# LoveDaisy/ice_halo_sim

Hardware: AMD Instinct MI355X
Metric: rays/sec (whole node) at 9 wavelengths, single-scatter hex column (higher is better)
Workload: dtype f32

## Files before the change

### ice_halo_sim_amd/csrc/halo_backend.cpp

```cpp
#include <cstdlib>
#include <dlfcn.h>
#include <hip/hip_runtime.h>

#include <algorithm>
#include <cmath>
#include <cstdio>
#include <cstring>
#include <map>
#include <memory>
#include <mutex>
#include <string>
#include <vector>

#include "halo_device.h"
#include "halo_host.hpp"
#include "halo_launch.h"

#ifndef HALO_XYZ_LOG_MIN_PIX
#define HALO_XYZ_LOG_MIN_PIX (1u << 19)
#endif

using namespace halo;

namespace {
// ... 47 lines not shown
  int mono_enabled = 1;
  int bin = -1;
  DevBuf<HitRec> bin_list_s[2], bin_list2_s[2];
  DevBuf<uint32_t> bin_cnt_s[2], bin_cnt2_s[2];
  int log_set = 0;
  Marker set_free[2];
  hipStream_t aux = nullptr;
  hipEvent_t ev_fork = nullptr, ev_join = nullptr;
  bool aux_pending = false;
  hipStream_t cs[2] = {nullptr, nullptr};
  hipEvent_t ev_cs[2] = {nullptr, nullptr}, ev_main = nullptr, ev_aux = nullptr;
  bool cs_pending[2] = {false, false};
  int cs_next = 0;
  uint64_t aux_seq = 0, cs_seen_aux[2] = {0, 0};
  int overlap = 1;
  int defer_fold = 0;
  int twin_set = 0;
  int lambda_planes = -1;
  int mono_copies = 8;
  uint32_t mono_s_log2 = 0;
  int blocks_per_cu = 24;
  int host_shapes = 0;
  int gen_serial = 0;
  int small_blocks_per_cu = 0;
  int blocks_cap = 0;
  int lazy_fold = 1;
  int hit_log = -1;
  uint32_t hit_log_cap = 0;
  int hex_fast = 1;
  int entry_fast = 1;
// ... 100 lines not shown
  uint64_t cont_in_n = 0;
  int cont_shuffle = 1;
  int cont_order = 0;
  DevBuf<uint32_t> cont_mask;
  DevBuf<uint32_t> cont_err;
  DevBuf<uint32_t> cont_base;
  DevBuf<uint32_t> cont_tiles;
  uint32_t cont_fill_max = 0;
  uint64_t cont_roots = 0;
  DevBuf<HaloExitRecord> exits;
  uint64_t exits_pending = 0;
  DevBuf<float> host_f;
  DevBuf<uint32_t> host_u;
  uint64_t sess_crystal_samples = 0, sess_orient_samples = 0;
  std::vector<hipEvent_t*> untimed_events() {
    return {&ev_cs[0], &ev_cs[1], &ev_main, &ev_aux, &ev_fork, &ev_join, &ev_gen, &ev_gate, &set_free[0].ev, &set_free[1].ev, &shapes_free[0].ev,
            &shapes_free[1].ev, &rmw[0].ev, &rmw[1].ev, &set_folded[0].ev, &set_folded[1].ev};
  }
};

namespace {

int fail(HaloBackend* b, int code, const std::string& msg) {
  if (b) b->error = msg;
  return code;
}
int hip_fail(HaloBackend* b, hipError_t e, const char* what) {
  return fail(b, (e == hipErrorNoDevice || e == hipErrorInvalidDevice || e == hipErrorOutOfMemory) ? HALO_UNAVAILABLE : HALO_FATAL,
              std::string(what) + ": " + hipGetErrorString(e));
}
#define HIPCHK(b, call)                                   \
// ... 17 lines not shown
  b->aux_seq++;
  return HALO_OK;
}
int join_aux(HaloBackend* b) {
  if (b->aux_pending) {
    HIPCHK(b, hipEventRecord(b->ev_join, b->aux));
    HIPCHK(b, hipStreamWaitEvent(b->stream, b->ev_join, 0));
    b->aux_pending = false;
  }
  for (int k = 0; k < 2; k++)
    if (b->cs_pending[k]) {
      HIPCHK(b, hipEventRecord(b->ev_cs[k], b->cs[k]));
      HIPCHK(b, hipStreamWaitEvent(b->stream, b->ev_cs[k], 0));
      b->cs_pending[k] = false;
      b->rmw[k].clear();
    }
  return HALO_OK;
}
int wait_for_aux(HaloBackend* b, int i) {
  if (b->overlap && b->aux_pending && b->cs_seen_aux[i] != b->aux_seq) {
    HIPCHK(b, hipEventRecord(b->ev_aux, b->aux));
    HIPCHK(b, hipStreamWaitEvent(b->cs[i], b->ev_aux, 0));
    b->cs_seen_aux[i] = b->aux_seq;
  }
  return HALO_OK;
}
int next_trace_stream(HaloBackend* b, bool touches_planes, bool alternate, hipStream_t* out, int* which) {
  if (!b->overlap) {
    *out = b->stream;
    *which = 0;
    return HALO_OK;
  }
  const int i = alternate ? b->cs_next : 0;
  if (alternate) b->cs_next ^= 1;
  HIPCHK(b, hipEventRecord(b->ev_main, b->stream));
  HIPCHK(b, hipStreamWaitEvent(b->cs[i], b->ev_main, 0));
  if (touches_planes)
    if (int rc = wait_for_aux(b, i)) return rc;
  b->cs_pending[i] = true;
// ... 240 lines not shown
  else if (k == "hit_log") b->hit_log = static_cast<int>(v);
  else if (k == "hit_log_cap") b->hit_log_cap = static_cast<uint32_t>(std::max<int64_t>(v, 0));
  else if (k == "gen_serial") b->gen_serial = v ? 1 : 0;
  else if (k == "shuffle_chunk") {
    if (v < 1 || v > 64 || (v & (v - 1)) != 0) return fail(b, HALO_FATAL, "shuffle_chunk must be a power of two in [1, 64]");
    b->shuffle_chunk_log2 = 0;
    while ((1ll << b->shuffle_chunk_log2) < v) b->shuffle_chunk_log2++;
  }
  else if (k == "lazy_fold") b->lazy_fold = v ? 1 : 0;
  else if (k == "table_cache") b->table_cache = v ? 1 : 0;
  else if (k == "overlap") {
    if (int rc = sync_all(b)) return rc;
    b->overlap = v ? 1 : 0;
  }
  else if (k == "defer_fold") b->defer_fold = v ? 1 : 0;
  else if (k == "gen_ahead") b->gen_ahead = v ? 1 : 0;
  else if (k == "pool_entry_fast") b->pool_entry_fast = v ? 1 : 0;
  else if (k == "rehit_strategy") {
    if (b->in_session) return fail(b, HALO_FATAL, "rehit_strategy cannot change inside a session");
    b->rehit_strategy = v ? 1 : 0;
  }
  else if (k == "cont_order") {
    if (b->in_session) return fail(b, HALO_FATAL, "cont_order cannot change inside a session");
    if (v != 0 && v != 1) return fail(b, HALO_FATAL, "cont_order must be 0 (append order) or 1 (canonical order)");
    b->cont_order = static_cast<int>(v);
  }
  else if (k == "log_tiles_log2") b->log_tiles_log2 = static_cast<int>(std::min<int64_t>(std::max<int64_t>(v, 0), 8));
  else if (k == "alt_log2") b->alt_log2 = static_cast<int>(std::min<int64_t>(std::max<int64_t>(v, 10), 28));
  else if (k == "small_blocks_per_cu") b->small_blocks_per_cu = static_cast<int>(std::max<int64_t>(v, 0));
  else if (k == "blocks_cap") b->blocks_cap = static_cast<int>(std::max<int64_t>(v, 0));
// ... 151 lines not shown
    const size_t one = (static_cast<size_t>(kMonoRows) << s_log2) * b->plane_copies * b->plane_cnt;
    b->mono_two = two_sets_n;
    b->mono_half = one;
    if (!b->mono_two) b->mono_set = 0;
    const size_t need = one * (b->mono_two ? 2u : 1u);
    if (b->mono.cap < need) {
      if (int rc = reserve_idle(b, b->mono, need)) return rc;
      HIPCHK(b, hipMemsetAsync(b->mono.ptr, 0, b->mono.cap * sizeof(float), b->stream));
    }
    b->mono_s_log2 = s_log2;
    const size_t twin_need = (static_cast<size_t>(kMonoRows) << s_log2) * b->plane_cnt;
    if (b->ovf.cap < 2u * twin_need && twin_need <= (512ull << 20)) {
      hipError_t oe = hipSuccess;
      if (int rc = reserve_idle(b, b->ovf, 2u * twin_need, &oe)) return rc;
      bool ok = oe == hipSuccess;
      if (ok && !b->ovf_flag.ptr) ok = b->ovf_flag.reserve(2) == hipSuccess && hipMemsetAsync(b->ovf_flag.ptr, 0, 2 * sizeof(uint32_t), b->stream) == hipSuccess;
      if (ok) {
        HIPCHK(b, hipMemsetAsync(b->ovf.ptr, 0, b->ovf.cap * sizeof(double), b->stream));
      } else {
        (void)hipGetLastError();
        b->ovf.release();
        b->ovf_flag.release();
      }
    }
  }
  if (!b->color_classes.empty()) {
    const size_t need = b->color_classes.size() * npix;
    if (b->lanes.cap < need || b->lanes_w != render->width || b->lanes_h != render->height) {
      if (int rc = reserve_idle(b, b->lanes, need)) return rc;
      if (int rc = join_aux(b)) return rc;
      HIPCHK(b, hipMemsetAsync(b->lanes.ptr, 0, b->lanes.cap * sizeof(double), b->stream));
// ... 17 lines not shown
  const double bound = 4.0 * std::max(max_w, 1e-30) * static_cast<double>(std::max<uint64_t>(m, 1));
  int e = 0;
  (void)std::frexp(bound, &e);
  return static_cast<uint32_t>(std::min(32, std::max(0, 62 - e)));
}

static double* twin_of(HaloBackend* b, int set) {
  const size_t half = (static_cast<size_t>(kMonoRows) << b->mono_s_log2) * b->plane_cnt;
  if (!b->ovf.ptr || !b->ovf_flag.ptr || b->ovf.cap < 2u * half) return nullptr;
  return b->ovf.ptr + static_cast<size_t>(set) * half;
}

static int fold_queue(HaloBackend* b) {
  if (!b->mono_dirty) return HALO_OK;
  HIPCHK(b, hipSetDevice(b->device));
  if (int rc = fork_aux(b)) return rc;
  hipStream_t ps = post_stream(b);
  const uint32_t npix = static_cast<uint32_t>(b->acc_w) * static_cast<uint32_t>(b->acc_h);
  const size_t plane = (static_cast<size_t>(kMonoRows) << b->mono_s_log2) * b->plane_copies;
  const size_t twin_plane = static_cast<size_t>(kMonoRows) << b->mono_s_log2;
  double* twin = twin_of(b, b->twin_set);
  uint32_t* flag = twin ? b->ovf_flag.ptr + b->twin_set : nullptr;
  for (uint32_t first = 0; first < b->plane_cnt; first += kFoldGroup) {
    const uint32_t n = std::min<uint32_t>(kFoldGroup, b->plane_cnt - first);
    FoldCoef coef{};
    for (uint32_t m = 0; m < n; m++)
      for (int a = 0; a < 3; a++) coef.c[m][a] = b->plane_coef[first + m][static_cast<size_t>(a)];
    hipError_t e = launch_fold(b->acc, planes_of(b) + first * plane, npix, b->mono_s_log2, b->plane_copies, n, coef, twin ? twin + first * twin_plane : nullptr, flag, ps);
    if (e != hipSuccess) return hip_fail(b, e, "halo_fold_kernel launch");
  }
  if (flag) HIPCHK(b, hipMemsetAsync(flag, 0, sizeof(uint32_t), ps));
  b->twin_set ^= 1;
  if (b->mono_two) {
    HIPCHK(b, b->set_folded[b->mono_set].mark(ps));
    b->mono_set ^= 1;
  }
  b->mono_dirty = false;
  return HALO_OK;
}
static int fold_if_dirty(HaloBackend* b) {
  if (int rc = fold_queue(b)) return rc;
  return join_aux(b);
}

int halo_end(halo_handle_t b) {
  if (!b) return HALO_FATAL;
// ... 312 lines not shown
  P.aggregate = static_cast<uint32_t>(b->aggregate);
  P.geom_clock = b->geom_clock;
  P.lanes = b->lanes.ptr;
  P.lane_stride = static_cast<uint32_t>(b->acc_w) * static_cast<uint32_t>(b->acc_h);
  return P;
}
int bind_route(HaloBackend* b, LaunchPlan& p, int ls, DispatchParams& P) {
  if (p.use_log)
    if (int rc = reserve_log_buffers(b, p, ls)) return rc;
  DevBuf<HitRec>&bin_list = b->bin_list_s[ls], &bin_list2 = b->bin_list2_s[ls];
  DevBuf<uint32_t>&bin_cnt = b->bin_cnt_s[ls], &bin_cnt2 = b->bin_cnt2_s[ls];
  if (p.use_bin)
    if (int rc = join_aux(b)) return rc;
  if (p.use_log) {
    if (int rc = reserve_idle(b, bin_cnt, std::max<size_t>(static_cast<size_t>(p.blocks), static_cast<size_t>(512) * 16u))) return rc;
    if (int rc = reserve_idle(b, bin_cnt2, static_cast<size_t>(512) * 16u)) return rc;
    HIPCHK(b, b->set_free[ls].wait_on(b->stream));
  } else if (p.use_bin) {
    if (int rc = reserve_idle(b, bin_cnt, static_cast<size_t>(512) * 16u)) return rc;
    HIPCHK(b, hipMemsetAsync(bin_cnt.ptr, 0, static_cast<size_t>(p.two_level ? 512u : p.bin_tiles) * 16u * sizeof(uint32_t), b->stream));
    if (int rc = reserve_idle(b, bin_list, p.cap1 * p.lists1)) return rc;
    if (p.two_level) {
      if (int rc = reserve_idle(b, bin_cnt2, static_cast<size_t>(p.bin_tiles) * 16u)) return rc;
      HIPCHK(b, hipMemsetAsync(bin_cnt2.ptr, 0, static_cast<size_t>(p.bin_tiles) * 16u * sizeof(uint32_t), b->stream));
      if (int rc = reserve_idle(b, bin_list2, p.cap2 * p.bin_tiles)) return rc;
    }
  }
  const bool lists = p.use_log || p.use_bin;
  P.bin_list = lists ? bin_list.ptr : nullptr;
  P.bin_log = p.use_log ? 1u : 0u;
  P.log_xyz = p.use_log_xyz ? 1u : 0u;
  P.mono_by_wl = b->mono_by_wl ? 1u : 0u;
  P.mono_copy_mask = lists ? 0u : b->plane_copies - 1u;
  if (lists) {
    P.bin_cap = static_cast<uint32_t>(p.cap1);
    P.bin_tiles = p.use_log ? p.log_tiles : p.two_level ? b->bin_l1 : p.bin_tiles;
    P.bin_shift = (p.use_bin && p.two_level) ? 14u + p.fan_log2 : 0u;
    P.bin_cnt = bin_cnt.ptr;
  }
// ... 40 lines not shown
      if (b->overlap && p.two_level) HIPCHK(b, b->rmw[ts_i].mark(ts));
    }
    HIPCHK(b, hipEventRecord(b->ring_ev1[k], ts));
    b->ring_posts[k] = false;
    HIPCHK(b, hipEventRecord(b->ring_done[k], ts));
    return HALO_OK;
  }
  HIPCHK(b, hipEventRecord(b->ring_ev1[k], ts));
  hipStream_t ps = ts;
  if (p.under_fold()) {
    if (b->mono_two) {
      HIPCHK(b, b->set_folded[b->mono_set].wait_on(ps));
    } else if (int rc = wait_for_aux(b, ts_i)) return rc;
  }
  HIPCHK(b, hipEventRecord(b->ring_ev2[k], ps));
  HIPCHK(b, hipMemsetAsync(bin_cnt2.ptr, 0, static_cast<size_t>(p.log_tiles) * 16u * sizeof(uint32_t), ps));
  hipError_t be = p.use_log_xyz ? launch_log_route_xyz(P.mono, P.log_plane_stride, bin_list.ptr, P.bin_cap, bin_cnt.ptr, static_cast<uint32_t>(p.blocks),
                                                       bin_list2.ptr, cap2, bin_cnt2.ptr, p.log_tiles, b->mono_s_log2, P.wl_pool, P.wl_pool_size, frac_bits, P.ovf, P.ovf_flag, P.ovf_copies_log2, ps, before_sums)
                                : launch_log_route(P.mono, bin_list.ptr, P.bin_cap, bin_cnt.ptr, static_cast<uint32_t>(p.blocks), bin_list2.ptr, cap2,
                                                   bin_cnt2.ptr, 1u << p.log_t_log2, p.log_planes, b->mono_s_log2, b->render.visible == HALO_VISIBLE_FULL, frac_bits,
                                                   P.ovf, P.ovf_flag, P.ovf_copies_log2, ps, before_sums);
  if (be != hipSuccess) return hip_fail(b, be, "halo_split_kernel launch");
  if (b->overlap) HIPCHK(b, b->rmw[ts_i].mark(ps));
  HIPCHK(b, hipEventRecord(b->ring_ev3[k], ps));
  HIPCHK(b, b->set_free[S.ls].mark(ps));
  if (b->overlap && p.alternate) b->log_set ^= 1;
  b->ring_posts[k] = true;
  HIPCHK(b, hipEventRecord(b->ring_done[k], ps));
  return HALO_OK;
}
int queue_launch(HaloBackend* b, const LaunchPlan& p, const HaloEntry& E, EntryTables& T, const DispatchParams& P, const LaunchSlots& S) {
  const int k = S.k;
  hipStream_t ts = nullptr;
  int ts_i = 0;
  if (int rc = next_trace_stream(b, !p.under_fold(), p.alternate, &ts, &ts_i)) return rc;
  hipEvent_t before_sums = nullptr;
#ifndef HALO_NO_PLANE_GATES
// ... 13 lines not shown
    if (ahead) {
      HIPCHK(b, hipEventRecord(b->ev_gen, gs));
      HIPCHK(b, hipStreamWaitEvent(ts, b->ev_gen, 0));
      b->cs_pending[1] = true;
    }
  }
  HIPCHK(b, hipEventRecord(b->ring_ev0[k], ts));
  b->ring_final[k] = P.final_layer != 0u;
  const int launch_geom = (p.geom == 0 && T.entry_fast && b->hex_fast && T.hex_regular) ? 3 : p.geom;
  hipError_t le = launch_trace(P, p.blocks, ts, T.mode, launch_geom, b->mono_session);
  if (T.ce) {
    T.ce->read_ring[T.ce->cur] = k;
    T.ce->read_use[T.ce->cur] = b->ring_use[k];
  }
  b->mono_dirty = true;
  record_route(b, p, P, T.mode, T.fast_mode, launch_geom);
  if (le != hipSuccess) return hip_fail(b, le, "halo_trace_kernel launch");
  if (!p.deterministic) HIPCHK(b, b->shapes_free[S.shape_set].mark(ts));
  if (int rc = queue_passes(b, p, P, S, ts, ts_i, before_sums)) return rc;
  b->tally_unread = true;
  b->ring_busy[k] = true;
  return HALO_OK;
}
int trace_launch(HaloBackend* b, const LayerCtx& c, LaunchPlan& p, EntryTables& T, DispatchParams& P) {
  const HaloEntry& E = b->scene.layers[c.layer].entries[p.ci];
  const uint64_t m = p.m;
  LaunchSlots S;
  std::vector<ShapeDev> pool((p.deterministic && !T.cached) || p.host_pool ? p.shape_cnt : 0u);
  for (uint32_t k = 0; k < static_cast<uint32_t>(pool.size()); k++) {
    if (c.host_crystal) host::ToShapeDev(*c.rays->crystal, pool[k]);
// ... 818 lines not shown
```

### ice_halo_sim_amd/csrc/halo_kernels.hip

```cpp
#include "halo_trace.inl"
#include "halo_launch.h"

namespace halo {

constexpr uint32_t kListOnceMin = 1u << 16;
template <bool ONCE>
__device__ __forceinline__ uint4 load_list_u4(const uint4* p) {
  if constexpr (!ONCE) return *p;
  const uint32_t* q = reinterpret_cast<const uint32_t*>(p);
  return make_uint4(__builtin_nontemporal_load(q), __builtin_nontemporal_load(q + 1), __builtin_nontemporal_load(q + 2), __builtin_nontemporal_load(q + 3));
}

struct FixQ {
  double to_fix, from_fix;
  __device__ __forceinline__ explicit FixQ(uint32_t frac_bits)
      : to_fix(__hiloint2double(static_cast<int>((1023u + frac_bits) << 20), 0)), from_fix(__hiloint2double(static_cast<int>((1023u - frac_bits) << 20), 0)) {}
  __device__ __forceinline__ unsigned long long fix(float v) const {
    return static_cast<unsigned long long>(static_cast<long long>(fma(static_cast<double>(fmaxf(v, 0.0f)), to_fix, 0.5)));
  }
  __device__ __forceinline__ float unfix(unsigned long long a) const { return static_cast<float>(static_cast<double>(a) * from_fix); }
};

constexpr int kBinBlock = 1024;
constexpr uint32_t kBinSplit = 2u;
// ... 173 lines not shown
        } else {
          for (uint32_t k = 0; k < 3u; ++k) c[k] = code == xyz.pool_size + k ? 1.0f : 0.0f;
        }
        const size_t at = r.x & slot_mask;
        for (uint32_t k = 0; k < 3u; ++k)
          if (c[k] != 0.0f) split_overflow(plane, xyz, at + static_cast<size_t>(k) * xyz.plane_stride, c[k] * __uint_as_float(r.y));
      } else {
        split_overflow(plane, xyz, r.x, __uint_as_float(r.y));
      }
    }
    __syncthreads();
  }
}

__global__ void __launch_bounds__(kBinBlock) halo_bin_accumulate_range_kernel(float* __restrict__ plane, const uint2* __restrict__ list, uint32_t cap,
                                                                               const uint32_t* __restrict__ cnt, uint32_t tile_log2, uint32_t frac_bits) {
  __shared__ __attribute__((aligned(16))) unsigned long long acc[1u << kBinTileLog2];
  const FixQ fq(frac_bits);
  const uint32_t tile = blockIdx.x;
  const uint32_t n = min(cnt[static_cast<size_t>(tile) * kBinCntStride], cap);
  if (n == 0u) return;
  const uint32_t slots = 1u << tile_log2, mask = slots - 1u;
  for (uint32_t j = threadIdx.x; j < slots; j += kBinBlock) acc[j] = 0ull;
  __syncthreads();
  const uint2* src = list + static_cast<size_t>(tile) * cap;
#ifndef HALO_ACC_U
#define HALO_ACC_U 4
#endif
  constexpr uint32_t kU = HALO_ACC_U;
  uint32_t i = threadIdx.x;
#ifndef HALO_ACC_NARROW
  const uint4* src4 = reinterpret_cast<const uint4*>(src);
  const uint32_t n2 = n / 2u;
  auto stream = [&](auto once) {
    for (; i + (kU - 1u) * kBinBlock < n2; i += kU * kBinBlock) {
      uint4 h[kU];
#pragma unroll
      for (uint32_t u = 0; u < kU; ++u) h[u] = load_list_u4<decltype(once)::value>(&src4[i + u * kBinBlock]);
#pragma unroll
// ... 30 lines not shown
  for (uint32_t j = threadIdx.x; j < slots / 4u; j += kBinBlock) {
    const float4 v = make_float4(fq.unfix(acc[4u * j]), fq.unfix(acc[4u * j + 1u]), fq.unfix(acc[4u * j + 2u]), fq.unfix(acc[4u * j + 3u]));
    if (v.x != 0.0f || v.y != 0.0f || v.z != 0.0f || v.w != 0.0f) {
      float4 q = dst[j];
      q.x += v.x;
      q.y += v.y;
      q.z += v.z;
      q.w += v.w;
      dst[j] = q;
    }
  }
}

template <uint32_t CH>
__global__ void __launch_bounds__(kBinBlock) halo_log_accumulate_kernel(float* __restrict__ planes, uint32_t plane_stride, const uint2* __restrict__ list, uint32_t cap,
                                                                        const uint32_t* __restrict__ cnt, const WlEntryDev* __restrict__ pool, uint32_t pool_size,
                                                                        uint32_t tiles_log2, uint32_t s_log2, uint32_t frac_bits) {
  constexpr uint32_t kTileLog2 = CH == 3u ? 12u : 14u;
  __shared__ __attribute__((aligned(16))) unsigned long long acc[CH][1u << kTileLog2];
  const FixQ fq(frac_bits);
  __shared__ __attribute__((aligned(16))) float s_cmf[CH == 3u ? HALO_WL_POOL_MAX + 3 : 1][4];
  const uint32_t tile = blockIdx.x;
  const uint32_t n = min(cnt[static_cast<size_t>(tile) * kBinCntStride], cap);
  if (n == 0u) return;
  const TileMap map{s_log2, tiles_log2};
  const uint32_t tile_in = tile & ((1u << tiles_log2) - 1u), plane_of_tile = tile >> tiles_log2, in_plane = (1u << (s_log2 + 10u)) - 1u;
  const uint32_t slots = 1u << (s_log2 + 10u - tiles_log2);
  for (uint32_t c = 0; c < CH; ++c)
    for (uint32_t j = threadIdx.x; j < slots; j += kBinBlock) acc[c][j] = 0ull;
  if constexpr (CH == 3u) {
    for (uint32_t j = threadIdx.x; j < pool_size + 3u; j += kBinBlock) {
      const bool unit = j >= pool_size;
      s_cmf[j][0] = unit ? (j == pool_size ? 1.0f : 0.0f) : pool[j].cmf_x;
      s_cmf[j][1] = unit ? (j == pool_size + 1u ? 1.0f : 0.0f) : pool[j].cmf_y;
      s_cmf[j][2] = unit ? (j == pool_size + 2u ? 1.0f : 0.0f) : pool[j].cmf_z;
      s_cmf[j][3] = 0.0f;
    }
  }
  __syncthreads();
  const uint2* src = list + static_cast<size_t>(tile) * cap;
  constexpr uint32_t kU = CH == 3u ? 8u : 4u, kSlotMask = CH == 3u ? (1u << kLogWlShift) - 1u : 0xFFFFFFFFu;
  auto add = [&](uint2 h) {
    uint32_t t_unused, s;
    map.split(h.x & kSlotMask & in_plane, t_unused, s);
    const float w = __uint_as_float(h.y);
    if constexpr (CH == 3u) {
      const uint32_t code = h.x >> kLogWlShift;
      const float4 c4 = *reinterpret_cast<const float4*>(s_cmf[code]);
      if (c4.x != 0.0f) atomicAdd(&acc[0][s], fq.fix(c4.x * w));
      if (c4.y != 0.0f) atomicAdd(&acc[1][s], fq.fix(c4.y * w));
      if (c4.z != 0.0f) atomicAdd(&acc[2][s], fq.fix(c4.z * w));
    } else {
      atomicAdd(&acc[0][s], fq.fix(w));
    }
// ... 39 lines not shown
    add(src[r]);
    if (r + 1u < n) add(src[r + 1u]);
  }
  __syncthreads();
  for (uint32_t c = 0; c < CH; ++c) {
    float* dst = planes + static_cast<size_t>(c) * plane_stride + (static_cast<size_t>(plane_of_tile) << (s_log2 + 10u));
    for (uint32_t j = threadIdx.x; j < slots; j += kBinBlock) {
      const float v = fq.unfix(acc[c][j]);
      if (v != 0.0f) dst[map.slot_of(tile_in, j)] += v;
    }
  }
}

hipError_t launch_log_route(float* plane, const HitRec* log, uint32_t cap1, const uint32_t* cnt1, uint32_t regions, HitRec* list2, uint32_t cap2, uint32_t* cnt2,
                            uint32_t tiles, uint32_t planes, uint32_t s_log2, bool interleaved, uint32_t frac_bits, double* ovf, uint32_t* ovf_flag, uint32_t copies_log2, hipStream_t stream,
                            hipEvent_t before_sums) {
  const uint32_t tiles_log2 = static_cast<uint32_t>(__builtin_ctz(tiles)), tile_log2 = s_log2 + 10u - tiles_log2;
  if (planes > 1u || tiles > 256u) {
    hipLaunchKernelGGL((halo_split_kernel<kLogSplitThreads, kLogSplitPer, 512u, false, true>), dim3(regions), dim3(kLogSplitThreads), 0, stream, plane, reinterpret_cast<const uint2*>(log), cap1, cnt1, 1u,
                       1u, reinterpret_cast<uint2*>(list2), cap2, cnt2, tiles_log2, 0u, 0xFFFFFFFFu, 0u, s_log2, SplitXyz{nullptr, 0u, 0u, ovf, ovf_flag, s_log2 + 10u, copies_log2});
    hipError_t e = hipGetLastError();
    if (e != hipSuccess) return e;
    if (before_sums && (e = hipStreamWaitEvent(stream, before_sums, 0)) != hipSuccess) return e;
    hipLaunchKernelGGL((halo_log_accumulate_kernel<1u>), dim3(tiles * planes), dim3(kBinBlock), 0, stream, plane, 0u, reinterpret_cast<const uint2*>(list2), cap2, cnt2,
                       static_cast<const WlEntryDev*>(nullptr), 0u, tiles_log2, s_log2, frac_bits);
    return hipGetLastError();
  }
  if (interleaved)
    hipLaunchKernelGGL((halo_split_kernel<kLogSplitThreads, kLogSplitPer, 256u, false, true>), dim3(regions), dim3(kLogSplitThreads), 0, stream, plane, reinterpret_cast<const uint2*>(log), cap1, cnt1, 1u,
                       1u, reinterpret_cast<uint2*>(list2), cap2, cnt2, tiles_log2, 0u, 0xFFFFFFFFu, 0u, s_log2, SplitXyz{nullptr, 0u, 0u, ovf, ovf_flag, s_log2 + 10u, copies_log2});
  else
    hipLaunchKernelGGL((halo_split_kernel<kLogSplitThreads, kLogSplitPer, 256u, false, false>), dim3(regions), dim3(kLogSplitThreads), 0, stream, plane, reinterpret_cast<const uint2*>(log), cap1, cnt1, 1u,
                       1u, reinterpret_cast<uint2*>(list2), cap2, cnt2, tiles_log2, 0u, 0xFFFFFFFFu, tile_log2, 0u, SplitXyz{nullptr, 0u, 0u, ovf, ovf_flag, s_log2 + 10u, copies_log2});
  hipError_t e = hipGetLastError();
  if (e != hipSuccess) return e;
  if (before_sums && (e = hipStreamWaitEvent(stream, before_sums, 0)) != hipSuccess) return e;
  if (interleaved)
    hipLaunchKernelGGL((halo_log_accumulate_kernel<1u>), dim3(tiles), dim3(kBinBlock), 0, stream, plane, 0u, reinterpret_cast<const uint2*>(list2), cap2, cnt2,
                       static_cast<const WlEntryDev*>(nullptr), 0u, tiles_log2, s_log2, frac_bits);
  else hipLaunchKernelGGL(halo_bin_accumulate_range_kernel, dim3(tiles), dim3(kBinBlock), 0, stream, plane, reinterpret_cast<const uint2*>(list2), cap2, cnt2, tile_log2, frac_bits);
  return hipGetLastError();
}

hipError_t launch_log_route_xyz(float* planes, uint32_t plane_stride, const HitRec* log, uint32_t cap1, const uint32_t* cnt1, uint32_t regions, HitRec* list2,
                                uint32_t cap2, uint32_t* cnt2, uint32_t tiles, uint32_t s_log2, const WlEntryDev* pool, uint32_t pool_size, uint32_t frac_bits,
                                double* ovf, uint32_t* ovf_flag, uint32_t copies_log2, hipStream_t stream, hipEvent_t before_sums) {
  const uint32_t tiles_log2 = static_cast<uint32_t>(__builtin_ctz(tiles));
  hipLaunchKernelGGL((halo_split_kernel<kLogSplitThreads, kLogSplitPer, 512u, true, true>), dim3(regions), dim3(kLogSplitThreads), 0, stream, planes, reinterpret_cast<const uint2*>(log), cap1, cnt1, 1u, 1u,
                     reinterpret_cast<uint2*>(list2), cap2, cnt2, tiles_log2, 0u, (1u << kLogWlShift) - 1u, 0u, s_log2, SplitXyz{pool, pool_size, plane_stride, ovf, ovf_flag, s_log2 + 10u, copies_log2});
  hipError_t e = hipGetLastError();
  if (e != hipSuccess) return e;
  if (before_sums && (e = hipStreamWaitEvent(stream, before_sums, 0)) != hipSuccess) return e;
  hipLaunchKernelGGL((halo_log_accumulate_kernel<3u>), dim3(tiles), dim3(kBinBlock), 0, stream, planes, plane_stride, reinterpret_cast<const uint2*>(list2), cap2, cnt2,
                     pool, pool_size, tiles_log2, s_log2, frac_bits);
  return hipGetLastError();
}

hipError_t launch_bin_two_level(float* plane, const HitRec* list1, uint32_t cap1, uint32_t* cnt1, uint32_t lists1, HitRec* list2, uint32_t cap2,
                                uint32_t* cnt2, uint32_t tiles, uint32_t fan_log2, uint32_t frac_bits, double* ovf, uint32_t* ovf_flag, hipStream_t stream, hipEvent_t before_sums) {
  hipLaunchKernelGGL((halo_split_kernel<256u, 16u, 256u, false, false>), dim3(lists1 * kSplitParts), dim3(256u), 0, stream, plane, reinterpret_cast<const uint2*>(list1), cap1,
                     cnt1, static_cast<uint32_t>(kBinCntStride), kSplitParts, reinterpret_cast<uint2*>(list2), cap2, cnt2, fan_log2, 1u, 0xFFFFFFFFu,
                     static_cast<uint32_t>(kBinTileLog2), 0u, SplitXyz{nullptr, 0u, 0u, ovf, ovf_flag, 0u, 0u});
  hipError_t e = hipGetLastError();
  if (e != hipSuccess) return e;
  if (before_sums && (e = hipStreamWaitEvent(stream, before_sums, 0)) != hipSuccess) return e;
  hipLaunchKernelGGL(halo_bin_accumulate_range_kernel, dim3(tiles), dim3(kBinBlock), 0, stream, plane, reinterpret_cast<const uint2*>(list2), cap2, cnt2,
                     static_cast<uint32_t>(kBinTileLog2), frac_bits);
  return hipGetLastError();
}

constexpr uint32_t kFoldTile = 64u;
constexpr uint32_t kFoldBatch = 8u;
template <uint32_t R>
__global__ void __launch_bounds__(kBlock) halo_fold_kernel(float* __restrict__ xyz, float* __restrict__ planes, uint32_t n_pix,
                                                            uint32_t s_log2, uint32_t copies, uint32_t n_planes, const FoldCoef coef,
                                                            double* __restrict__ ovf, const uint32_t* __restrict__ ovf_flag) {
  __shared__ float tile[3][R][kFoldTile + 1];
  const bool take_ovf = ovf != nullptr && *ovf_flag != 0u;
  const uint32_t tiles_c = (1u << s_log2) / kFoldTile;
  const uint32_t row0 = (blockIdx.x / tiles_c) * R, col0 = (blockIdx.x % tiles_c) * kFoldTile;
  const size_t plane = static_cast<size_t>(kMonoRows) << s_log2;
  const uint32_t lo = threadIdx.x & (kFoldTile - 1u), hi = threadIdx.x / kFoldTile;
  for (uint32_t r = hi; r < R; r += kBlock / kFoldTile) {
    float* q = planes + (static_cast<size_t>(row0 + r) << s_log2) + col0 + lo;
    float x = 0.0f, y = 0.0f, z = 0.0f;
    if (copies == 1u) {
      for (uint32_t p0 = 0; p0 < n_planes; p0 += kFoldBatch) {
        float t[kFoldBatch];
#pragma unroll
        for (uint32_t u = 0; u < kFoldBatch; ++u) t[u] = p0 + u < n_planes ? q[static_cast<size_t>(p0 + u) * plane] : 0.0f;
        if (take_ovf) {
// ... 52 lines not shown
  }
  __syncthreads();
  const uint32_t s_mask = (1u << s_log2) - 1u;
  const uint32_t wr = threadIdx.x % R;
  for (uint32_t c = threadIdx.x / R; c < kFoldTile; c += kBlock / R) {
    const float x = tile[0][wr][c], y = tile[1][wr][c], z = tile[2][wr][c];
    if (x == 0.0f && y == 0.0f && z == 0.0f) continue;
    const uint32_t a = ((col0 + c) * kMonoMulInv) & s_mask;
    const uint32_t pix = a * kMonoRows + row0 + wr;
    if (pix < n_pix) {
      xyz[3u * pix + 0u] += x;
      xyz[3u * pix + 1u] += y;
      xyz[3u * pix + 2u] += z;
    }
  }
}

__global__ void __launch_bounds__(kBlock) halo_consumer_fold_kernel(float* __restrict__ acc, float* __restrict__ sum,
                                                                     float* __restrict__ comp, uint32_t n) {
  const uint32_t stride = gridDim.x * kBlock;
  for (uint32_t i = blockIdx.x * kBlock + threadIdx.x; i < n; i += stride) {
    const float delta = acc[i];
    if (delta == 0.0f) continue;
    acc[i] = 0.0f;
    const float s = sum[i];
    const float ns = s + delta;
    comp[i] += (fabsf(delta) < fabsf(s)) ? ((s - ns) + delta) : ((delta - ns) + s);
    sum[i] = ns;
  }
}
// ... 179 lines not shown
}

hipError_t launch_post_snapshot(const float* sum, const float* comp, uint8_t* rgb_out, float* xyz_out, uint32_t n_pix, float scale,
                                const float ray_color[3], const float background[3], int blocks, hipStream_t stream) {
  DisplayDev d;
  d.scale = scale;
  for (int j = 0; j < 3; j++) {
    d.ray_color[j] = ray_color[j];
    d.background[j] = background[j];
  }
  hipLaunchKernelGGL(halo_post_snapshot_kernel, dim3(blocks), dim3(kBlock), 0, stream, sum, comp, rgb_out, xyz_out, n_pix, d);
  return hipGetLastError();
}

hipError_t launch_fold(float* xyz, float* planes, uint32_t n_pix, uint32_t s_log2, uint32_t copies, uint32_t n_planes, const FoldCoef& coef,
                       double* ovf, const uint32_t* ovf_flag, hipStream_t stream) {
  const uint32_t tiles_c = (1u << s_log2) / kFoldTile;
  if (tiles_c * (kMonoRows / 64u) >= 512u)
    hipLaunchKernelGGL(halo_fold_kernel<64u>, dim3(tiles_c * (kMonoRows / 64u)), dim3(kBlock), 0, stream, xyz, planes, n_pix, s_log2, copies, n_planes, coef, ovf, ovf_flag);
  else if (tiles_c * (kMonoRows / 16u) >= 512u)
    hipLaunchKernelGGL(halo_fold_kernel<16u>, dim3(tiles_c * (kMonoRows / 16u)), dim3(kBlock), 0, stream, xyz, planes, n_pix, s_log2, copies, n_planes, coef, ovf, ovf_flag);
  else
    hipLaunchKernelGGL(halo_fold_kernel<4u>, dim3(tiles_c * (kMonoRows / 4u)), dim3(kBlock), 0, stream, xyz, planes, n_pix, s_log2, copies, n_planes, coef, ovf, ovf_flag);
  return hipGetLastError();
}

constexpr uint32_t kScanBlock = 256u, kScanItems = 8u, kScanTile = kScanBlock * kScanItems;

__device__ __forceinline__ uint32_t wave_inclusive_scan(uint32_t v) {
  const uint32_t lane = __lane_id();
#pragma unroll
  for (uint32_t d = 1u; d < 64u; d <<= 1) {
    const uint32_t t = __shfl_up(v, d, 64);
    if (lane >= d) v += t;
  }
  return v;
}
__device__ __forceinline__ uint32_t block_exclusive_scan(uint32_t v, uint32_t& total) {
// ... 134 lines not shown
```

### ice_halo_sim_amd/csrc/halo_launch.h

```cpp
#ifndef HALO_LAUNCH_H_
#define HALO_LAUNCH_H_

#include <hip/hip_runtime.h>

#include "halo_device.h"

namespace halo {
namespace geom {
struct CrystalRecipe;
}

hipError_t launch_trace(const DispatchParams& P, int blocks, hipStream_t stream, int mode, int geom, bool mono);
hipError_t launch_bin_accumulate(float* plane, const HitRec* list, uint32_t cap, uint32_t* cnt, uint32_t tiles, uint32_t frac_bits, hipStream_t stream);
hipError_t launch_bin_two_level(float* plane, const HitRec* list1, uint32_t cap1, uint32_t* cnt1, uint32_t lists1, HitRec* list2, uint32_t cap2,
                                uint32_t* cnt2, uint32_t tiles, uint32_t fan_log2, uint32_t frac_bits, double* ovf, uint32_t* ovf_flag, hipStream_t stream, hipEvent_t before_sums);
hipError_t launch_log_route(float* plane, const HitRec* log, uint32_t cap1, const uint32_t* cnt1, uint32_t regions, HitRec* list2, uint32_t cap2, uint32_t* cnt2,
                            uint32_t tiles, uint32_t planes, uint32_t s_log2, bool interleaved, uint32_t frac_bits, double* ovf, uint32_t* ovf_flag, uint32_t copies_log2, hipStream_t stream,
                            hipEvent_t before_sums);
hipError_t launch_log_route_xyz(float* planes, uint32_t plane_stride, const HitRec* log, uint32_t cap1, const uint32_t* cnt1, uint32_t regions, HitRec* list2,
                                uint32_t cap2, uint32_t* cnt2, uint32_t tiles, uint32_t s_log2, const WlEntryDev* pool, uint32_t pool_size, uint32_t frac_bits,
                                double* ovf, uint32_t* ovf_flag, uint32_t copies_log2, hipStream_t stream, hipEvent_t before_sums);
hipError_t launch_shapegen(void* pool, bool prism_records, uint32_t n, uint32_t seed, const geom::CrystalRecipe& rc, uint64_t first_index,
                           hipStream_t stream, bool serial_pyramid);
hipError_t launch_fold(float* xyz, float* planes, uint32_t n_pix, uint32_t s_log2, uint32_t copies, uint32_t n_planes, const FoldCoef& coef,
                       double* ovf, const uint32_t* ovf_flag, hipStream_t stream);
hipError_t launch_consumer_fold(float* acc, float* sum, float* comp, uint32_t n, int blocks, hipStream_t stream);
hipError_t launch_lane_hist(const double* lanes, uint32_t n_pix, const CompositeDev& cd, uint32_t shift, uint32_t bits, uint32_t prefix, uint32_t* hist, int blocks,
                            hipStream_t stream);
hipError_t launch_composite(const double* lanes, uint32_t n_pix, const CompositeDev& cd, float* rgb_out, uint8_t* srgb_out, int blocks, hipStream_t stream);
hipError_t launch_lanes_load(const float* src, double* lanes, uint64_t n, int blocks, hipStream_t stream);
hipError_t launch_lanes_drain(double* lanes, float* dst, uint64_t n, int blocks, hipStream_t stream);
hipError_t launch_lanes_add(const float* src, double* lanes, uint64_t n, int blocks, hipStream_t stream);
hipError_t launch_post_snapshot(const float* sum, const float* comp, uint8_t* rgb_out, float* xyz_out, uint32_t n_pix, float scale,
                                const float ray_color[3], const float background[3], int blocks, hipStream_t stream);
hipError_t launch_cont_reorder(const float* in, uint32_t in_stride, uint32_t region, const uint32_t* cnt, uint32_t max_fill, const uint32_t* mask, uint32_t n_roots,
                               uint32_t* tile_sum, uint32_t* base, float* out, uint32_t out_stride, uint32_t n_cont, uint32_t planes, uint32_t* err, hipStream_t stream);

}

#endif
// ... 1 lines not shown
```

Measured before the change: 25.38 billion.

## Clear bin counters in-kernel and run session-tail fold on the trace stream

The accumulate kernels now zero their per-tile second-level counters themselves, so the per-batch memset on the trace stream is replaced by a one-time full clear. The final fold kernel resets the overflow flag through a last-block atomic counter instead of a separate memset. When the last trace ran on trace stream 0, the fold is queued on that stream rather than forked onto the auxiliary stream, with new event plumbing so stream 1 waits for it. The aim is to remove small memset launches and cross-stream fork/join overhead at the session tail, at the cost of more complex stream-ordering state that could race if an ordering edge is missed.

```diff
diff --git a/ice_halo_sim_amd/csrc/halo_backend.cpp b/ice_halo_sim_amd/csrc/halo_backend.cpp
--- a/ice_halo_sim_amd/csrc/halo_backend.cpp
+++ b/ice_halo_sim_amd/csrc/halo_backend.cpp
@@ -85,6 +85,11 @@
   int cs_next = 0;
   uint64_t aux_seq = 0, cs_seen_aux[2] = {0, 0};
   int overlap = 1;
+  int session_tail = 1;
+  bool cnt2_clean[2] = {false, false};
+  bool last_kept_stream0 = false;
+  bool tfold_pending = false;
+  hipEvent_t ev_tfold = nullptr;
   int defer_fold = 0;
   int twin_set = 0;
   int lambda_planes = -1;
@@ -215,7 +220,7 @@
   DevBuf<uint32_t> host_u;
   uint64_t sess_crystal_samples = 0, sess_orient_samples = 0;
   std::vector<hipEvent_t*> untimed_events() {
-    return {&ev_cs[0], &ev_cs[1], &ev_main, &ev_aux, &ev_fork, &ev_join, &ev_gen, &ev_gate, &set_free[0].ev, &set_free[1].ev, &shapes_free[0].ev,
+    return {&ev_cs[0], &ev_cs[1], &ev_main, &ev_aux, &ev_fork, &ev_join, &ev_gen, &ev_gate, &ev_tfold, &set_free[0].ev, &set_free[1].ev, &shapes_free[0].ev,
             &shapes_free[1].ev, &rmw[0].ev, &rmw[1].ev, &set_folded[0].ev, &set_folded[1].ev};
   }
 };
@@ -263,6 +268,7 @@
       HIPCHK(b, hipStreamWaitEvent(b->stream, b->ev_cs[k], 0));
       b->cs_pending[k] = false;
       b->rmw[k].clear();
+      if (k == 0) b->tfold_pending = false;
     }
   return HALO_OK;
 }
@@ -272,6 +278,23 @@
     HIPCHK(b, hipStreamWaitEvent(b->cs[i], b->ev_aux, 0));
     b->cs_seen_aux[i] = b->aux_seq;
   }
+  if (b->overlap && i == 1 && b->tfold_pending) {
+    HIPCHK(b, hipEventRecord(b->ev_tfold, b->cs[0]));
+    HIPCHK(b, hipStreamWaitEvent(b->cs[1], b->ev_tfold, 0));
+    b->tfold_pending = false;
+  }
+  return HALO_OK;
+}
+int fork_trace(HaloBackend* b) {
+  HIPCHK(b, hipEventRecord(b->ev_fork, b->stream));
+  HIPCHK(b, hipStreamWaitEvent(b->cs[0], b->ev_fork, 0));
+  if (b->cs_pending[1]) {
+    HIPCHK(b, hipEventRecord(b->ev_cs[1], b->cs[1]));
+    HIPCHK(b, hipStreamWaitEvent(b->cs[0], b->ev_cs[1], 0));
+  }
+  if (int rc = wait_for_aux(b, 0)) return rc;
+  b->cs_pending[0] = true;
+  b->tfold_pending = true;
   return HALO_OK;
 }
 int next_trace_stream(HaloBackend* b, bool touches_planes, bool alternate, hipStream_t* out, int* which) {
@@ -542,6 +565,11 @@
     b->overlap = v ? 1 : 0;
   }
   else if (k == "defer_fold") b->defer_fold = v ? 1 : 0;
+  else if (k == "session_tail") {
+    if (b->in_session) return fail(b, HALO_FATAL, "session_tail cannot change inside a session");
+    if (v != 0 && v != 1) return fail(b, HALO_FATAL, "session_tail must be 0 (fills and auxiliary-stream folds) or 1 (kernels clear counters and flag; trace-stream fold)");
+    b->session_tail = static_cast<int>(v);
+  }
   else if (k == "gen_ahead") b->gen_ahead = v ? 1 : 0;
   else if (k == "pool_entry_fast") b->pool_entry_fast = v ? 1 : 0;
   else if (k == "rehit_strategy") {
@@ -723,7 +751,7 @@
       hipError_t oe = hipSuccess;
       if (int rc = reserve_idle(b, b->ovf, 2u * twin_need, &oe)) return rc;
       bool ok = oe == hipSuccess;
-      if (ok && !b->ovf_flag.ptr) ok = b->ovf_flag.reserve(2) == hipSuccess && hipMemsetAsync(b->ovf_flag.ptr, 0, 2 * sizeof(uint32_t), b->stream) == hipSuccess;
+      if (ok && !b->ovf_flag.ptr) ok = b->ovf_flag.reserve(4) == hipSuccess && hipMemsetAsync(b->ovf_flag.ptr, 0, 4 * sizeof(uint32_t), b->stream) == hipSuccess;
       if (ok) {
         HIPCHK(b, hipMemsetAsync(b->ovf.ptr, 0, b->ovf.cap * sizeof(double), b->stream));
       } else {
@@ -771,22 +799,25 @@
 static int fold_queue(HaloBackend* b) {
   if (!b->mono_dirty) return HALO_OK;
   HIPCHK(b, hipSetDevice(b->device));
-  if (int rc = fork_aux(b)) return rc;
-  hipStream_t ps = post_stream(b);
+  const bool on_trace = b->session_tail != 0 && b->overlap != 0 && b->last_kept_stream0;
+  if (int rc = on_trace ? fork_trace(b) : fork_aux(b)) return rc;
+  hipStream_t ps = on_trace ? b->cs[0] : post_stream(b);
   const uint32_t npix = static_cast<uint32_t>(b->acc_w) * static_cast<uint32_t>(b->acc_h);
   const size_t plane = (static_cast<size_t>(kMonoRows) << b->mono_s_log2) * b->plane_copies;
   const size_t twin_plane = static_cast<size_t>(kMonoRows) << b->mono_s_log2;
   double* twin = twin_of(b, b->twin_set);
   uint32_t* flag = twin ? b->ovf_flag.ptr + b->twin_set : nullptr;
+  uint32_t* done = (flag && b->session_tail != 0) ? b->ovf_flag.ptr + 2 + b->twin_set : nullptr;
   for (uint32_t first = 0; first < b->plane_cnt; first += kFoldGroup) {
     const uint32_t n = std::min<uint32_t>(kFoldGroup, b->plane_cnt - first);
     FoldCoef coef{};
     for (uint32_t m = 0; m < n; m++)
       for (int a = 0; a < 3; a++) coef.c[m][a] = b->plane_coef[first + m][static_cast<size_t>(a)];
-    hipError_t e = launch_fold(b->acc, planes_of(b) + first * plane, npix, b->mono_s_log2, b->plane_copies, n, coef, twin ? twin + first * twin_plane : nullptr, flag, ps);
+    hipError_t e = launch_fold(b->acc, planes_of(b) + first * plane, npix, b->mono_s_log2, b->plane_copies, n, coef, twin ? twin + first * twin_plane : nullptr, flag, ps,
+                               first + kFoldGroup >= b->plane_cnt ? done : nullptr);
     if (e != hipSuccess) return hip_fail(b, e, "halo_fold_kernel launch");
   }
-  if (flag) HIPCHK(b, hipMemsetAsync(flag, 0, sizeof(uint32_t), ps));
+  if (flag && !done) HIPCHK(b, hipMemsetAsync(flag, 0, sizeof(uint32_t), ps));
   b->twin_set ^= 1;
   if (b->mono_two) {
     HIPCHK(b, b->set_folded[b->mono_set].mark(ps));
@@ -1129,7 +1160,9 @@
     if (int rc = join_aux(b)) return rc;
   if (p.use_log) {
     if (int rc = reserve_idle(b, bin_cnt, std::max<size_t>(static_cast<size_t>(p.blocks), static_cast<size_t>(512) * 16u))) return rc;
+    const uint32_t* had = bin_cnt2.ptr;
     if (int rc = reserve_idle(b, bin_cnt2, static_cast<size_t>(512) * 16u)) return rc;
+    if (bin_cnt2.ptr != had) b->cnt2_clean[ls] = false;
     HIPCHK(b, b->set_free[ls].wait_on(b->stream));
   } else if (p.use_bin) {
     if (int rc = reserve_idle(b, bin_cnt, static_cast<size_t>(512) * 16u)) return rc;
@@ -1138,6 +1171,7 @@
     if (p.two_level) {
       if (int rc = reserve_idle(b, bin_cnt2, static_cast<size_t>(p.bin_tiles) * 16u)) return rc;
       HIPCHK(b, hipMemsetAsync(bin_cnt2.ptr, 0, static_cast<size_t>(p.bin_tiles) * 16u * sizeof(uint32_t), b->stream));
+      b->cnt2_clean[ls] = false;
       if (int rc = reserve_idle(b, bin_list2, p.cap2 * p.bin_tiles)) return rc;
     }
   }
@@ -1208,13 +1242,17 @@
     } else if (int rc = wait_for_aux(b, ts_i)) return rc;
   }
   HIPCHK(b, hipEventRecord(b->ring_ev2[k], ps));
-  HIPCHK(b, hipMemsetAsync(bin_cnt2.ptr, 0, static_cast<size_t>(p.log_tiles) * 16u * sizeof(uint32_t), ps));
+  const bool clear_cnt = b->session_tail != 0;
+  if (!clear_cnt) HIPCHK(b, hipMemsetAsync(bin_cnt2.ptr, 0, static_cast<size_t>(p.log_tiles) * 16u * sizeof(uint32_t), ps));
+  else if (!b->cnt2_clean[S.ls]) HIPCHK(b, hipMemsetAsync(bin_cnt2.ptr, 0, bin_cnt2.cap * sizeof(uint32_t), ps));
+  b->cnt2_clean[S.ls] = false;
   hipError_t be = p.use_log_xyz ? launch_log_route_xyz(P.mono, P.log_plane_stride, bin_list.ptr, P.bin_cap, bin_cnt.ptr, static_cast<uint32_t>(p.blocks),
-                                                       bin_list2.ptr, cap2, bin_cnt2.ptr, p.log_tiles, b->mono_s_log2, P.wl_pool, P.wl_pool_size, frac_bits, P.ovf, P.ovf_flag, P.ovf_copies_log2, ps, before_sums)
+                                                       bin_list2.ptr, cap2, bin_cnt2.ptr, p.log_tiles, b->mono_s_log2, P.wl_pool, P.wl_pool_size, frac_bits, P.ovf, P.ovf_flag, P.ovf_copies_log2, ps, before_sums, clear_cnt)
                                 : launch_log_route(P.mono, bin_list.ptr, P.bin_cap, bin_cnt.ptr, static_cast<uint32_t>(p.blocks), bin_list2.ptr, cap2,
                                                    bin_cnt2.ptr, 1u << p.log_t_log2, p.log_planes, b->mono_s_log2, b->render.visible == HALO_VISIBLE_FULL, frac_bits,
-                                                   P.ovf, P.ovf_flag, P.ovf_copies_log2, ps, before_sums);
+                                                   P.ovf, P.ovf_flag, P.ovf_copies_log2, ps, before_sums, clear_cnt);
   if (be != hipSuccess) return hip_fail(b, be, "halo_split_kernel launch");
+  b->cnt2_clean[S.ls] = clear_cnt;
   if (b->overlap) HIPCHK(b, b->rmw[ts_i].mark(ps));
   HIPCHK(b, hipEventRecord(b->ring_ev3[k], ps));
   HIPCHK(b, b->set_free[S.ls].mark(ps));
@@ -1258,6 +1296,7 @@
     T.ce->read_use[T.ce->cur] = b->ring_use[k];
   }
   b->mono_dirty = true;
+  b->last_kept_stream0 = b->overlap != 0 && !p.alternate;
   record_route(b, p, P, T.mode, T.fast_mode, launch_geom);
   if (le != hipSuccess) return hip_fail(b, le, "halo_trace_kernel launch");
   if (!p.deterministic) HIPCHK(b, b->shapes_free[S.shape_set].mark(ts));
diff --git a/ice_halo_sim_amd/csrc/halo_kernels.hip b/ice_halo_sim_amd/csrc/halo_kernels.hip
--- a/ice_halo_sim_amd/csrc/halo_kernels.hip
+++ b/ice_halo_sim_amd/csrc/halo_kernels.hip
@@ -211,7 +211,7 @@
 }
 
 __global__ void __launch_bounds__(kBinBlock) halo_bin_accumulate_range_kernel(float* __restrict__ plane, const uint2* __restrict__ list, uint32_t cap,
-                                                                               const uint32_t* __restrict__ cnt, uint32_t tile_log2, uint32_t frac_bits) {
+                                                                               uint32_t* __restrict__ cnt, uint32_t tile_log2, uint32_t frac_bits, uint32_t clear_cnt) {
   __shared__ __attribute__((aligned(16))) unsigned long long acc[1u << kBinTileLog2];
   const FixQ fq(frac_bits);
   const uint32_t tile = blockIdx.x;
@@ -220,6 +220,7 @@
   const uint32_t slots = 1u << tile_log2, mask = slots - 1u;
   for (uint32_t j = threadIdx.x; j < slots; j += kBinBlock) acc[j] = 0ull;
   __syncthreads();
+  if (clear_cnt != 0u && threadIdx.x == 0u) cnt[static_cast<size_t>(tile) * kBinCntStride] = 0u;
   const uint2* src = list + static_cast<size_t>(tile) * cap;
 #ifndef HALO_ACC_U
 #define HALO_ACC_U 4
@@ -280,8 +281,8 @@
 
 template <uint32_t CH>
 __global__ void __launch_bounds__(kBinBlock) halo_log_accumulate_kernel(float* __restrict__ planes, uint32_t plane_stride, const uint2* __restrict__ list, uint32_t cap,
-                                                                        const uint32_t* __restrict__ cnt, const WlEntryDev* __restrict__ pool, uint32_t pool_size,
-                                                                        uint32_t tiles_log2, uint32_t s_log2, uint32_t frac_bits) {
+                                                                        uint32_t* __restrict__ cnt, const WlEntryDev* __restrict__ pool, uint32_t pool_size,
+                                                                        uint32_t tiles_log2, uint32_t s_log2, uint32_t frac_bits, uint32_t clear_cnt) {
   constexpr uint32_t kTileLog2 = CH == 3u ? 12u : 14u;
   __shared__ __attribute__((aligned(16))) unsigned long long acc[CH][1u << kTileLog2];
   const FixQ fq(frac_bits);
@@ -304,6 +305,7 @@
     }
   }
   __syncthreads();
+  if (clear_cnt != 0u && threadIdx.x == 0u) cnt[static_cast<size_t>(tile) * kBinCntStride] = 0u;
   const uint2* src = list + static_cast<size_t>(tile) * cap;
   constexpr uint32_t kU = CH == 3u ? 8u : 4u, kSlotMask = CH == 3u ? (1u << kLogWlShift) - 1u : 0xFFFFFFFFu;
   auto add = [&](uint2 h) {
@@ -373,7 +375,8 @@
 
 hipError_t launch_log_route(float* plane, const HitRec* log, uint32_t cap1, const uint32_t* cnt1, uint32_t regions, HitRec* list2, uint32_t cap2, uint32_t* cnt2,
                             uint32_t tiles, uint32_t planes, uint32_t s_log2, bool interleaved, uint32_t frac_bits, double* ovf, uint32_t* ovf_flag, uint32_t copies_log2, hipStream_t stream,
-                            hipEvent_t before_sums) {
+                            hipEvent_t before_sums, bool clear_cnt) {
+  const uint32_t clr = clear_cnt ? 1u : 0u;
   const uint32_t tiles_log2 = static_cast<uint32_t>(__builtin_ctz(tiles)), tile_log2 = s_log2 + 10u - tiles_log2;
   if (planes > 1u || tiles > 256u) {
     hipLaunchKernelGGL((halo_split_kernel<kLogSplitThreads, kLogSplitPer, 512u, false, true>), dim3(regions), dim3(kLogSplitThreads), 0, stream, plane, reinterpret_cast<const uint2*>(log), cap1, cnt1, 1u,
@@ -382,7 +385,7 @@
     if (e != hipSuccess) return e;
     if (before_sums && (e = hipStreamWaitEvent(stream, before_sums, 0)) != hipSuccess) return e;
     hipLaunchKernelGGL((halo_log_accumulate_kernel<1u>), dim3(tiles * planes), dim3(kBinBlock), 0, stream, plane, 0u, reinterpret_cast<const uint2*>(list2), cap2, cnt2,
-                       static_cast<const WlEntryDev*>(nullptr), 0u, tiles_log2, s_log2, frac_bits);
+                       static_cast<const WlEntryDev*>(nullptr), 0u, tiles_log2, s_log2, frac_bits, clr);
     return hipGetLastError();
   }
   if (interleaved)
@@ -396,14 +399,14 @@
   if (before_sums && (e = hipStreamWaitEvent(stream, before_sums, 0)) != hipSuccess) return e;
   if (interleaved)
     hipLaunchKernelGGL((halo_log_accumulate_kernel<1u>), dim3(tiles), dim3(kBinBlock), 0, stream, plane, 0u, reinterpret_cast<const uint2*>(list2), cap2, cnt2,
-                       static_cast<const WlEntryDev*>(nullptr), 0u, tiles_log2, s_log2, frac_bits);
-  else hipLaunchKernelGGL(halo_bin_accumulate_range_kernel, dim3(tiles), dim3(kBinBlock), 0, stream, plane, reinterpret_cast<const uint2*>(list2), cap2, cnt2, tile_log2, frac_bits);
+                       static_cast<const WlEntryDev*>(nullptr), 0u, tiles_log2, s_log2, frac_bits, clr);
+  else hipLaunchKernelGGL(halo_bin_accumulate_range_kernel, dim3(tiles), dim3(kBinBlock), 0, stream, plane, reinterpret_cast<const uint2*>(list2), cap2, cnt2, tile_log2, frac_bits, clr);
   return hipGetLastError();
 }
 
 hipError_t launch_log_route_xyz(float* planes, uint32_t plane_stride, const HitRec* log, uint32_t cap1, const uint32_t* cnt1, uint32_t regions, HitRec* list2,
                                 uint32_t cap2, uint32_t* cnt2, uint32_t tiles, uint32_t s_log2, const WlEntryDev* pool, uint32_t pool_size, uint32_t frac_bits,
-                                double* ovf, uint32_t* ovf_flag, uint32_t copies_log2, hipStream_t stream, hipEvent_t before_sums) {
+                                double* ovf, uint32_t* ovf_flag, uint32_t copies_log2, hipStream_t stream, hipEvent_t before_sums, bool clear_cnt) {
   const uint32_t tiles_log2 = static_cast<uint32_t>(__builtin_ctz(tiles));
   hipLaunchKernelGGL((halo_split_kernel<kLogSplitThreads, kLogSplitPer, 512u, true, true>), dim3(regions), dim3(kLogSplitThreads), 0, stream, planes, reinterpret_cast<const uint2*>(log), cap1, cnt1, 1u, 1u,
                      reinterpret_cast<uint2*>(list2), cap2, cnt2, tiles_log2, 0u, (1u << kLogWlShift) - 1u, 0u, s_log2, SplitXyz{pool, pool_size, plane_stride, ovf, ovf_flag, s_log2 + 10u, copies_log2});
@@ -411,7 +414,7 @@
   if (e != hipSuccess) return e;
   if (before_sums && (e = hipStreamWaitEvent(stream, before_sums, 0)) != hipSuccess) return e;
   hipLaunchKernelGGL((halo_log_accumulate_kernel<3u>), dim3(tiles), dim3(kBinBlock), 0, stream, planes, plane_stride, reinterpret_cast<const uint2*>(list2), cap2, cnt2,
-                     pool, pool_size, tiles_log2, s_log2, frac_bits);
+                     pool, pool_size, tiles_log2, s_log2, frac_bits, clear_cnt ? 1u : 0u);
   return hipGetLastError();
 }
 
@@ -424,7 +427,7 @@
   if (e != hipSuccess) return e;
   if (before_sums && (e = hipStreamWaitEvent(stream, before_sums, 0)) != hipSuccess) return e;
   hipLaunchKernelGGL(halo_bin_accumulate_range_kernel, dim3(tiles), dim3(kBinBlock), 0, stream, plane, reinterpret_cast<const uint2*>(list2), cap2, cnt2,
-                     static_cast<uint32_t>(kBinTileLog2), frac_bits);
+                     static_cast<uint32_t>(kBinTileLog2), frac_bits, 0u);
   return hipGetLastError();
 }
 
@@ -433,7 +436,7 @@
 template <uint32_t R>
 __global__ void __launch_bounds__(kBlock) halo_fold_kernel(float* __restrict__ xyz, float* __restrict__ planes, uint32_t n_pix,
                                                             uint32_t s_log2, uint32_t copies, uint32_t n_planes, const FoldCoef coef,
-                                                            double* __restrict__ ovf, const uint32_t* __restrict__ ovf_flag) {
+                                                            double* __restrict__ ovf, uint32_t* ovf_flag, uint32_t* done) {
   __shared__ float tile[3][R][kFoldTile + 1];
   const bool take_ovf = ovf != nullptr && *ovf_flag != 0u;
   const uint32_t tiles_c = (1u << s_log2) / kFoldTile;
@@ -516,6 +519,13 @@
       xyz[3u * pix + 2u] += z;
     }
   }
+  if (done != nullptr && threadIdx.x == 0u) {
+    __threadfence();
+    if (atomicAdd(done, 1u) == gridDim.x - 1u) {
+      *ovf_flag = 0u;
+      *done = 0u;
+    }
+  }
 }
 
 __global__ void __launch_bounds__(kBlock) halo_consumer_fold_kernel(float* __restrict__ acc, float* __restrict__ sum,
@@ -725,14 +735,16 @@
 }
 
 hipError_t launch_fold(float* xyz, float* planes, uint32_t n_pix, uint32_t s_log2, uint32_t copies, uint32_t n_planes, const FoldCoef& coef,
-                       double* ovf, const uint32_t* ovf_flag, hipStream_t stream) {
+                       double* ovf, const uint32_t* ovf_flag, hipStream_t stream, uint32_t* done) {
   const uint32_t tiles_c = (1u << s_log2) / kFoldTile;
+  uint32_t* flag = const_cast<uint32_t*>(ovf_flag);
+  if (ovf_flag == nullptr) done = nullptr;
   if (tiles_c * (kMonoRows / 64u) >= 512u)
-    hipLaunchKernelGGL(halo_fold_kernel<64u>, dim3(tiles_c * (kMonoRows / 64u)), dim3(kBlock), 0, stream, xyz, planes, n_pix, s_log2, copies, n_planes, coef, ovf, ovf_flag);
+    hipLaunchKernelGGL(halo_fold_kernel<64u>, dim3(tiles_c * (kMonoRows / 64u)), dim3(kBlock), 0, stream, xyz, planes, n_pix, s_log2, copies, n_planes, coef, ovf, flag, done);
   else if (tiles_c * (kMonoRows / 16u) >= 512u)
-    hipLaunchKernelGGL(halo_fold_kernel<16u>, dim3(tiles_c * (kMonoRows / 16u)), dim3(kBlock), 0, stream, xyz, planes, n_pix, s_log2, copies, n_planes, coef, ovf, ovf_flag);
+    hipLaunchKernelGGL(halo_fold_kernel<16u>, dim3(tiles_c * (kMonoRows / 16u)), dim3(kBlock), 0, stream, xyz, planes, n_pix, s_log2, copies, n_planes, coef, ovf, flag, done);
   else
-    hipLaunchKernelGGL(halo_fold_kernel<4u>, dim3(tiles_c * (kMonoRows / 4u)), dim3(kBlock), 0, stream, xyz, planes, n_pix, s_log2, copies, n_planes, coef, ovf, ovf_flag);
+    hipLaunchKernelGGL(halo_fold_kernel<4u>, dim3(tiles_c * (kMonoRows / 4u)), dim3(kBlock), 0, stream, xyz, planes, n_pix, s_log2, copies, n_planes, coef, ovf, flag, done);
   return hipGetLastError();
 }
 
diff --git a/ice_halo_sim_amd/csrc/halo_launch.h b/ice_halo_sim_amd/csrc/halo_launch.h
--- a/ice_halo_sim_amd/csrc/halo_launch.h
+++ b/ice_halo_sim_amd/csrc/halo_launch.h
@@ -16,14 +16,14 @@
                                 uint32_t* cnt2, uint32_t tiles, uint32_t fan_log2, uint32_t frac_bits, double* ovf, uint32_t* ovf_flag, hipStream_t stream, hipEvent_t before_sums);
 hipError_t launch_log_route(float* plane, const HitRec* log, uint32_t cap1, const uint32_t* cnt1, uint32_t regions, HitRec* list2, uint32_t cap2, uint32_t* cnt2,
                             uint32_t tiles, uint32_t planes, uint32_t s_log2, bool interleaved, uint32_t frac_bits, double* ovf, uint32_t* ovf_flag, uint32_t copies_log2, hipStream_t stream,
-                            hipEvent_t before_sums);
+                            hipEvent_t before_sums, bool clear_cnt = false);
 hipError_t launch_log_route_xyz(float* planes, uint32_t plane_stride, const HitRec* log, uint32_t cap1, const uint32_t* cnt1, uint32_t regions, HitRec* list2,
                                 uint32_t cap2, uint32_t* cnt2, uint32_t tiles, uint32_t s_log2, const WlEntryDev* pool, uint32_t pool_size, uint32_t frac_bits,
-                                double* ovf, uint32_t* ovf_flag, uint32_t copies_log2, hipStream_t stream, hipEvent_t before_sums);
+                                double* ovf, uint32_t* ovf_flag, uint32_t copies_log2, hipStream_t stream, hipEvent_t before_sums, bool clear_cnt = false);
 hipError_t launch_shapegen(void* pool, bool prism_records, uint32_t n, uint32_t seed, const geom::CrystalRecipe& rc, uint64_t first_index,
                            hipStream_t stream, bool serial_pyramid);
 hipError_t launch_fold(float* xyz, float* planes, uint32_t n_pix, uint32_t s_log2, uint32_t copies, uint32_t n_planes, const FoldCoef& coef,
-                       double* ovf, const uint32_t* ovf_flag, hipStream_t stream);
+                       double* ovf, const uint32_t* ovf_flag, hipStream_t stream, uint32_t* done = nullptr);
 hipError_t launch_consumer_fold(float* acc, float* sum, float* comp, uint32_t n, int blocks, hipStream_t stream);
 hipError_t launch_lane_hist(const double* lanes, uint32_t n_pix, const CompositeDev& cd, uint32_t shift, uint32_t bits, uint32_t prefix, uint32_t* hist, int blocks,
                             hipStream_t stream);
```

Result: no change. 25.32 billion (-0.2%).
